# eBay/Sequence-Semantic-Embedding

Measured on AMD Instinct MI355X. Metric: encoded seqs/sec (+ query x target cosine-scores/sec, top-1 vs ref), higher is better.
Workload: dtype f32; 1 GPU; configs[1]: classification stand-in, dual-encoder LSTM H=S=256 E=50 T=32 V=32000; encode 16384 source seqs/GPU/step + cosine top-10 vs 571-target index; batch_per_gpu=16384, seq_len=32, targets=571, parallelism=dp1, weights=random-init (reference initialisers, seed 0)

## Files before the change

### sequence-semantic-embedding_amd/csrc/lstm_fwd.hip

```cpp
#include <cstdlib>
#include <type_traits>

#include "sse_kernels.h"

#define LSTM_THREADS 512
#define LSTM_BM 64

#ifdef SSE_FWD_CLOCK
#include <cstdio>
__device__ long long g_fwd_clk[16 * 8];
#define FW_CLK_DECL long long ck_[8] = {0, 0, 0, 0, 0, 0, 0, 0}, ck_t = clock64();
#define FW_CLK(i)                   \
  {                                 \
    const long long n_ = clock64(); \
    ck_[i] += n_ - ck_t;            \
    ck_t = n_;                      \
  }
#else
#define FW_CLK_DECL
#define FW_CLK(i)
#endif

bool lstm_fwd_x_double(int KGx, int KGh, int RT) { return (size_t)(2 * RT * (KGx + KGh) + 1) * 1024 <= 160 * 1024; }
size_t lstm_fwd_lds_bytes(int KGx, int KGh, int RT) {
  const int xb = lstm_fwd_x_double(KGx, KGh, RT) ? 2 : 1;
  return (size_t)(xb * RT * KGx + 2 * RT * KGh) * 256 * sizeof(float) + 64 * 4 * sizeof(float);
}
static size_t lstm_fwd_xt_lds_bytes(int KGh, int RT) { return (size_t)(2 * RT * KGh) * 256 * sizeof(float) + 64 * 4 * sizeof(float); }


typedef unsigned int u32x4 __attribute__((ext_vector_type(4)));

__device__ __forceinline__ f32x4 wload(__amdgpu_buffer_rsrc_t r, int voff, int soff) {
  return __builtin_bit_cast(f32x4, __builtin_amdgcn_raw_buffer_load_b128(r, voff, soff, 0));
}

struct NoTail {
  __device__ void operator()() const {}
};
template <int MT, bool LIN, bool SWAP, int R = (MT == 1 ? 4 : 3), bool PRIO = true, typename Tail = NoTail>
__device__ __forceinline__ void gemm_pass(__amdgpu_buffer_rsrc_t wr, int voff, int soff, const float *const (&xa)[MT],
                                          const float *const (&ha)[MT], int KGx, int kend, f32x16 (&acc)[MT][2], int kbeg = 0,
                                          const Tail &tail = Tail{}) {
  auto a_frag = [&](int m, int kg) -> f32x4 {
    if constexpr (LIN) return *reinterpret_cast<const f32x4 *>(xa[m] + kg * 256);
    return *reinterpret_cast<const f32x4 *>(kg < KGx ? xa[m] + kg * 256 : ha[m] + (kg - KGx) * 256);
  };
  f32x4 p0[R], p1[R], af[R][MT];
  const int klast = kend - 1;
#pragma unroll
  for (int s = 0; s < R; ++s) {
    const int kg = kbeg + s < kend ? kbeg + s : klast;
    p0[s] = wload(wr, voff, soff + kg * 4096);
    p1[s] = wload(wr, voff + 1024, soff + kg * 4096);
#pragma unroll
    for (int m = 0; m < MT; ++m) af[s][m] = a_frag(m, kg);
    __builtin_amdgcn_sched_barrier(0);
  }
  auto mfmas = [&](int s) {
#pragma unroll
    for (int e = 0; e < 4; ++e)
#pragma unroll
      for (int m = 0; m < MT; ++m) {
        acc[m][0] = SWAP ? __builtin_amdgcn_mfma_f32_32x32x2f32(p0[s][e], af[s][m][e], acc[m][0], 0, 0, 0)
                         : __builtin_amdgcn_mfma_f32_32x32x2f32(af[s][m][e], p0[s][e], acc[m][0], 0, 0, 0);
        acc[m][1] = SWAP ? __builtin_amdgcn_mfma_f32_32x32x2f32(p1[s][e], af[s][m][e], acc[m][1], 0, 0, 0)
                         : __builtin_amdgcn_mfma_f32_32x32x2f32(af[s][m][e], p1[s][e], acc[m][1], 0, 0, 0);
      }
  };
  if constexpr (PRIO) __builtin_amdgcn_s_setprio(1);
  int kg = kbeg;
  for (; kg + R <= kend; kg += R) {
#pragma unroll
    for (int s = 0; s < R; ++s) {
      __builtin_amdgcn_sched_barrier(0);
      mfmas(s);
      __builtin_amdgcn_sched_barrier(0);
      const int kn = (kg + s + R < kend) ? kg + s + R : klast;
      p0[s] = wload(wr, voff, soff + kn * 4096);
      p1[s] = wload(wr, voff + 1024, soff + kn * 4096);
#pragma unroll
      for (int m = 0; m < MT; ++m) af[s][m] = a_frag(m, kn);
    }
  }
  if constexpr (!std::is_same_v<Tail, NoTail>) {
    __builtin_amdgcn_sched_barrier(0);
    tail();
    __builtin_amdgcn_sched_barrier(0);
  }
#pragma unroll
  for (int s = 0; s < R - 1; ++s)
    if (kg + s < kend) mfmas(s);
  if constexpr (PRIO) __builtin_amdgcn_s_setprio(0);
}

template <int RT, int MT, int UBW, bool TRAIN, bool LIN, bool SPL = false, bool TSW = false, bool XT = false>
__global__ __launch_bounds__(LSTM_THREADS) void lstm_fwd_kernel(LstmFwdArgs a) {
  static_assert(!TSW || TRAIN, "TSW is the training forward in the inference orientation");
  static_assert(!XT || (!TRAIN && LIN && !SPL), "the x table is an inference path of the linear LDS layout");
  constexpr int NTHR = LSTM_THREADS;
  extern __shared__ __attribute__((aligned(16))) float smem[];
  constexpr int ROWS = RT * 32;
  constexpr int TPR = NTHR / ROWS;
  constexpr int NWR = 8 / RT;
  constexpr bool SWAP = !TRAIN || TSW;
  const int tid = threadIdx.x, lane = tid & 63, w = tid >> 6;
  const bool split3 = !TRAIN && RT == 2 && MT == 1 && a.H > 64 && a.H <= 96;
  int ub0 = (RT == 2 && MT == 1) ? (w >> 1) : w;
  int mt0 = (RT == 2 && MT == 1) ? (w & 1) : 0;
  bool do_a = true, do_b = true;
  if (split3 && w >= 4) {
    ub0 = 2;
    mt0 = (w - 4) >> 1;
    do_a = ((w & 1) == 0);
    do_b = !do_a;
  }
  if constexpr (SPL) {
    static_assert(RT == 1 && MT == 1 && UBW == 1, "pass-split mapping is defined for one 32-row tile");
    ub0 = w & 3;
    do_a = w < 4;
    do_b = !do_a;
  }
  const int fidx = SPL ? ub0 : mt0;
  const int KGx = a.KGx, KGh = a.KGh, KG = KGx + KGh, T = a.T;
  const int KGhe = (a.KGhe > 0 && a.KGhe < KGh) ? a.KGhe : KGh;
  const int KGxs = XT ? 0 : KGx, KGs = KGxs + KGh;
  constexpr bool XD = LIN;
  auto xptr = [&](int buf, int mt) -> float * {
    return LIN ? smem + (size_t)((buf * RT + mt) * KGs) * 256 : smem + (size_t)(mt * KGx) * 256;
  };
  auto hptr = [&](int buf, int mt) -> float * {
    return LIN ? smem + (size_t)((buf * RT + mt) * KGs + KGxs) * 256
               : smem + (size_t)(RT * KGx + (buf * RT + mt) * KGh) * 256;
  };
  float *red = smem + (size_t)(LIN ? 2 * RT * KGs : RT * KGx + 2 * RT * KGh) * 256;
  const int b0 = blockIdx.x * ROWS;
  int *pass_flag = reinterpret_cast<int *>(red + 16);
  if (tid < 8) pass_flag[tid] = 0;

  const int xr = tid % ROWS, xq = tid / ROWS;
  const bool row_ok = (b0 + xr) < a.B;
  const int32_t *id_row = a.ids + (size_t)(row_ok ? (a.row_map ? a.row_map[b0 + xr] : b0 + xr) : 0) * T;
  auto fetch_id = [&](int t) -> int {
    int id = row_ok ? id_row[t] : 0;
    if (id < 0 || id >= a.V) {
      atomicOr(a.err, 1);
      id = 0;
    }
    return id;
  };
  int xt_row[MT];
#pragma unroll
  for (int m = 0; m < MT; ++m) {
    const int r = b0 + (mt0 + m) * 32 + (lane & 31);
    xt_row[m] = XT && r < a.B ? (a.row_map ? a.row_map[r] : r) : -1;
  }
  auto xt_id = [&](int m, int t) -> int { return xt_row[m] >= 0 ? a.ids[(size_t)xt_row[m] * T + t] : 0; };
  auto xt_check = [&](int id) -> int {
    if (id < 0 || id >= a.V) {
      atomicOr(a.err, 1);
      id = 0;
    }
    return id;
  };
  auto x_store = [&](int buf, int kg, f32x4 lo, f32x4 hi) {
    float *dst = xptr(buf, xr >> 5) + (size_t)kg * 256;
    *reinterpret_cast<f32x4 *>(dst + (xr & 31) * 4) = lo;
    *reinterpret_cast<f32x4 *>(dst + (32 + (xr & 31)) * 4) = hi;
  };

  const int NT32 = a.NT32 > 0 ? a.NT32 : gridDim.x * RT;
  auto tape_x = [&](int ts, int kg, f32x4 lo, f32x4 hi) {
    if constexpr (TSW) {
      if (kg >= 8) return;
      sse_quad_transpose(lo, lane);
      sse_quad_transpose(hi, lane);
      const int KT = 2 + KGh / 4, b = xr & 31;
      const size_t rg = ((size_t)ts * NT32 + blockIdx.x * RT + (xr >> 5)) * 4 + (b >> 3);
      const int k0 = kg * 8 + (xr & 3);
      float *dst = a.tape_a + (rg * KT + (k0 >> 5)) * 256 + ((((b >> 2) & 1) * 32 + (k0 & 31)) << 2);
      __builtin_nontemporal_store(lo, reinterpret_cast<f32x4 *>(dst));
      __builtin_nontemporal_store(hi, reinterpret_cast<f32x4 *>(dst + 16));
    }
  };

  int t0 = 0;
  if (!TRAIN && a.pad_h != nullptr) {
    int lead = T;
    if (row_ok) {
      for (int t = xq; t < T; t += TPR)
        if (id_row[t] != 0) {
          lead = t;
          break;
        }
    }
#pragma unroll
    for (int o = 32; o > 0; o >>= 1) lead = min(lead, __shfl_xor(lead, o));
    if (lane == 0) red[w] = __int_as_float(lead);
    __syncthreads();
    lead = T;
    for (int i = 0; i < NTHR / 64; ++i) lead = min(lead, __float_as_int(red[i]));
    t0 = min(lead, T - 1);
    __syncthreads();
  }

  int xid[MT];
#pragma unroll
  for (int m = 0; m < MT; ++m) xid[m] = XT ? xt_check(xt_id(m, t0)) : 0;
  if constexpr (!XT) {
    const int id = fetch_id(t0);
    const float *src = a.emb + (size_t)id * a.Ep;
    for (int kg = xq; kg < KGx; kg += TPR) {
      f32x4 lo = *reinterpret_cast<const f32x4 *>(src + kg * 8);
      f32x4 hi = *reinterpret_cast<const f32x4 *>(src + kg * 8 + 4);
      x_store(t0 & 1, kg, lo, hi);
    }
    if constexpr (TSW) {
      for (int kg = xq; kg < 8; kg += TPR) {
        f32x4 lo = {0, 0, 0, 0}, hi = {0, 0, 0, 0};
        if (kg < KGx) {
          lo = *reinterpret_cast<const f32x4 *>(src + kg * 8);
          hi = *reinterpret_cast<const f32x4 *>(src + kg * 8 + 4);
        }
        tape_x(t0, kg, lo, hi);
      }
    }
  }
  {
    const int Hp = KGh * 8;
    for (int i = tid; i < RT * KGh * 256; i += NTHR) {
      const int mt = i / (KGh * 256), e = i % (KGh * 256);
      const int un = (e >> 8) * 8 + ((e >> 7) & 1) * 4 + (e & 3);
      hptr(t0 & 1, mt)[e] = (t0 > 0) ? a.pad_h[(size_t)t0 * Hp + un] : 0.0f;
    }
  }

  f32x16 c[UBW][MT];
#pragma unroll
  for (int u = 0; u < UBW; ++u) {
#pragma unroll
    for (int r = 0; r < 16; ++r) {
      const int un = (ub0 + 8 * u) * 32 + (SWAP ? mfma_row(r, lane) : (lane & 31));
      const float c0 = (t0 > 0) ? a.pad_c[(size_t)t0 * (KGh * 8) + un] : 0.0f;
#pragma unroll
      for (int m = 0; m < MT; ++m) c[u][m][r] = c0;
    }
  }

  if constexpr (TSW) {
    if (do_b) {
      const int KT = 2 + KGh / 4, b = lane & 31;
#pragma unroll
      for (int u = 0; u < UBW; ++u)
#pragma unroll
        for (int m = 0; m < MT; ++m) {
          const size_t rg = ((size_t)t0 * NT32 + blockIdx.x * RT + mt0 + m) * 4 + (b >> 3);
#pragma unroll
          for (int q4 = 0; q4 < 4; ++q4) {
            float *dst = a.tape_a + (rg * KT + 2 + ub0 + 8 * u) * 256 + ((((b >> 2) & 1) * 32 + q4 * 8 + (lane >> 5) * 4 + (b & 3)) << 2);
            __builtin_nontemporal_store(f32x4{0, 0, 0, 0}, reinterpret_cast<f32x4 *>(dst));
          }
        }
    }
  }
  __syncthreads();

  const __amdgpu_buffer_rsrc_t wr = __builtin_amdgcn_make_buffer_rsrc(
      const_cast<float *>(a.Wp), 0, (KGh / 4) * KG * 4096, 0x00020000);
  const int wvoff = lane * 16;
  const __amdgpu_buffer_rsrc_t xtr = __builtin_amdgcn_make_buffer_rsrc(
      const_cast<float *>(a.xtab), 0, XT ? a.V * a.xtab_ub * 512 : 0, 0x00020000);
  auto xt_load = [&](f32x16(&acc)[MT][2], const int (&id)[MT], int ub, int q) {
    const int soff = __builtin_amdgcn_readfirstlane(ub * 512 + q * 128);
#pragma unroll
    for (int m = 0; m < MT; ++m) {
      const int voff = id[m] * (a.xtab_ub * 512) + (lane >> 5) * 64;
#pragma unroll
      for (int i = 0; i < 4; ++i) {
        const f32x4 v0 = wload(xtr, voff + 16 * i, soff), v1 = wload(xtr, voff + 128 + 16 * i, soff);
#pragma unroll
        for (int e = 0; e < 4; ++e) {
          acc[m][0][4 * i + e] = v0[e];
          acc[m][1][4 * i + e] = v1[e];
        }
      }
    }
  };

  auto acc_init = [&](f32x16(&acc)[MT][2], const int (&id)[MT], int ub, int q) {
    if constexpr (XT) {
      xt_load(acc, id, ub, q);
    } else {
#pragma unroll
      for (int m = 0; m < MT; ++m)
#pragma unroll
        for (int r = 0; r < 16; ++r) {
          acc[m][0][r] = 0.0f;
          acc[m][1][r] = 0.0f;
        }
    }
  };

  constexpr bool PF = XT && RT == 2 && MT == 2 && UBW == 1;
  const bool live0 = !(a.H > 0 && ub0 * 32 >= a.H);
  f32x16 ga[MT][2], gb[MT][2];
  if (PF && live0) xt_load(ga, xid, ub0, 0);

  FW_CLK_DECL
  for (int t = t0; t < T; ++t) {
    FW_CLK(0)
    const bool have_next = (t + 1) < T;
    int nid = 0;
    f32x4 nlo = {0, 0, 0, 0}, nhi = {0, 0, 0, 0};
    int xnid[MT];
#pragma unroll
    for (int m = 0; m < MT; ++m) xnid[m] = XT && have_next ? xt_id(m, t + 1) : 0;
    if (!XT && have_next) {
      nid = fetch_id(t + 1);
      if (xq < KGx) {
        const float *src = a.emb + (size_t)nid * a.Ep + xq * 8;
        nlo = *reinterpret_cast<const f32x4 *>(src);
        nhi = *reinterpret_cast<const f32x4 *>(src + 4);
      }
    }

    const int cur = t & 1, nxt = (t + 1) & 1;
    const float *xa[MT], *ha[MT];
#pragma unroll
    for (int m = 0; m < MT; ++m) {
      xa[m] = xptr(cur, mt0 + m) + lane * 4;
      ha[m] = hptr(cur, mt0 + m) + lane * 4;
    }

    if constexpr (TRAIN && !TSW) {
      const int KT = 2 + KGh / 4;
      const int nk = 64 + KGh * 8;
      auto a_elem = [&](int mt, int kp, int b) -> float {
        if (kp >= 64) {
          const int un = kp - 64;
          return hptr(cur, mt)[(size_t)(un >> 3) * 256 + ((((un >> 2) & 1) * 32 + b) << 2) + (un & 3)];
        }
        if (kp < KGx * 8) return xptr(cur, mt)[(size_t)(kp >> 3) * 256 + ((((kp >> 2) & 1) * 32 + b) << 2) + (kp & 3)];
        return 0.0f;
      };
      if (a.tape_a_split) {
        unsigned short *ta = reinterpret_cast<unsigned short *>(a.tape_a);
        for (int i = tid; i < nk * (ROWS / 8); i += NTHR) {
          const int kp = i % nk, o = i / nk;
          const int mt = o >> 2, oc = o & 3;
          float v8[8];
#pragma unroll
          for (int e = 0; e < 8; ++e) v8[e] = a_elem(mt, kp, oc * 8 + e);
          sse_u32x4 hi, lo;
          sse_split8(v8, hi, lo);
          const size_t g16 = ((size_t)t * NT32 + blockIdx.x * RT + mt) * 2 + (oc >> 1);
          unsigned short *dst = ta + ((g16 * KT + (kp >> 5)) * 2) * 512 + ((oc & 1) * 32 + (kp & 31)) * 8;
          *reinterpret_cast<sse_u32x4 *>(dst) = hi;
          *reinterpret_cast<sse_u32x4 *>(dst + 512) = lo;
        }
      } else {
        for (int i = tid; i < nk * (ROWS / 4); i += NTHR) {
          const int kp = i % nk, b4 = i / nk;
          const int mt = b4 >> 3, bl = (b4 & 7) * 4;
          const f32x4 v = {a_elem(mt, kp, bl), a_elem(mt, kp, bl + 1), a_elem(mt, kp, bl + 2), a_elem(mt, kp, bl + 3)};
          const size_t rg = ((size_t)t * NT32 + blockIdx.x * RT + mt) * 4 + (bl >> 3);
          float *dst = a.tape_a + (rg * KT + (kp >> 5)) * 256 + ((((bl >> 2) & 1) * 32 + (kp & 31)) << 2);
          *reinterpret_cast<f32x4 *>(dst) = v;
        }
      }
    }
    const int kend = (t == 0) ? KGx : KGx + KGhe;

#pragma unroll
    for (int u = 0; u < UBW; ++u) {
      const int ub = ub0 + 8 * u;
      if (!TRAIN && a.H > 0 && ub * 32 >= a.H) {
        if (u == 0 && XD && !XT && have_next) {
          if (xq < KGx) x_store(nxt, xq, nlo, nhi);
          for (int kg = xq + TPR; kg < KGx; kg += TPR) {
            const float *src = a.emb + (size_t)nid * a.Ep + kg * 8;
            x_store(nxt, kg, *reinterpret_cast<const f32x4 *>(src), *reinterpret_cast<const f32x4 *>(src + 4));
          }
        }
        continue;
      }
      const int unit = ub * 32 + (lane & 31);
      const int hoff = SWAP ? (ub * 4) * 256 + lane * 4
                            : (unit >> 3) * 256 + ((((unit >> 2) & 1) * 32) << 2) + (unit & 3);
      const int wsoff = __builtin_amdgcn_readfirstlane(ub) * KG * 4096;
      float *tp[MT];
      if constexpr (TRAIN) {
#pragma unroll
        for (int m = 0; m < MT; ++m)
          tp[m] = a.tape_g + (((size_t)t * NT32 + blockIdx.x * RT + mt0 + m) * (KGh / 4) + ub) * 5 * 1024 + lane * 4;
      }

      float *hdst[MT];
      auto pass = [&](int soff, f32x16(&acc)[MT][2], const auto &tail) {
        if constexpr (XT) {
          if (t > 0) gemm_pass<MT, true, SWAP>(wr, wvoff, soff + KGx * 4096, ha, ha, 0, KGhe, acc, 0, tail);
          else tail();
        } else {
          gemm_pass<MT, LIN, SWAP>(wr, wvoff, soff, xa, ha, KGx, kend, acc);
        }
      };
      auto tail_a = [&] {
        if constexpr (PF) xt_load(gb, xid, ub, 2);
      };
      auto tail_b = [&] {
        if constexpr (PF) {
          if (u + 1 < UBW && (a.H <= 0 || (ub + 8) * 32 < a.H)) {
            xt_load(ga, xid, ub + 8, 0);
          } else if (have_next) {
#pragma unroll
            for (int m = 0; m < MT; ++m) xid[m] = xt_check(xnid[m]);
            xt_load(ga, xid, ub0, 0);
          } else {
#pragma unroll
            for (int m = 0; m < MT; ++m)
#pragma unroll
              for (int r = 0; r < 16; ++r) ga[m][0][r] = ga[m][1][r] = 0.0f;
          }
        }
      };
#pragma unroll
      for (int m = 0; m < MT; ++m) hdst[m] = hptr(nxt, mt0 + m) + hoff;
      if (!PF && (!XT || do_a)) acc_init(ga, xid, ub, 0);
      FW_CLK(1)
      if (do_a) pass(wsoff, ga, tail_a);
      FW_CLK(2)
#pragma unroll
      for (int m = 0; m < MT; ++m) {
        if (!do_a) break;
        if constexpr (SWAP) {
#pragma unroll
          for (int q4 = 0; q4 < 4; ++q4) {
            f32x4 pij, si4, tj4;
#pragma unroll
            for (int e = 0; e < 4; ++e) {
              si4[e] = sse_sigmoid(ga[m][0][q4 * 4 + e]);
              tj4[e] = sse_tanh(ga[m][1][q4 * 4 + e]);
              pij[e] = si4[e] * tj4[e];
            }
            *reinterpret_cast<f32x4 *>(hdst[m] + q4 * 256) = pij;
            if constexpr (TSW) {
              __builtin_nontemporal_store(si4, reinterpret_cast<f32x4 *>(tp[m] + q4 * 256));
              __builtin_nontemporal_store(tj4, reinterpret_cast<f32x4 *>(tp[m] + 1024 + q4 * 256));
            }
          }
        } else {
#pragma unroll
          for (int q4 = 0; q4 < 4; ++q4) {
            f32x4 si4, tj4;
#pragma unroll
            for (int e = 0; e < 4; ++e) {
              const int r = q4 * 4 + e;
              si4[e] = sse_sigmoid(ga[m][0][r]);
              tj4[e] = sse_tanh(ga[m][1][r]);
              hdst[m][mfma_row(r, lane) << 2] = si4[e] * tj4[e];
            }
            if constexpr (TRAIN) {
              __builtin_nontemporal_store(si4, reinterpret_cast<f32x4 *>(tp[m] + q4 * 256));
              __builtin_nontemporal_store(tj4, reinterpret_cast<f32x4 *>(tp[m] + 1024 + q4 * 256));
            }
          }
        }
      }
      if (do_a && !do_b) {
        __builtin_amdgcn_s_waitcnt(0xc07f);
        if (lane == 0) __hip_atomic_store(pass_flag + fidx, t + 1, __ATOMIC_RELAXED, __HIP_MEMORY_SCOPE_WORKGROUP);
      }
      if (u == 0 && XD && !XT && have_next) {
        if (xq < KGx) x_store(nxt, xq, nlo, nhi);
        for (int kg = xq + TPR; kg < KGx; kg += TPR) {
          const float *src = a.emb + (size_t)nid * a.Ep + kg * 8;
          x_store(nxt, kg, *reinterpret_cast<const f32x4 *>(src), *reinterpret_cast<const f32x4 *>(src + 4));
        }
        tape_x(t + 1, xq, nlo, nhi);
      }
      if (!PF && (!XT || do_b)) acc_init(gb, xid, ub, 2);
      FW_CLK(3)
      if (do_b) pass(wsoff + 2048, gb, tail_b);
      FW_CLK(4)
      if (do_b && !do_a) {
        while (__hip_atomic_load(pass_flag + fidx, __ATOMIC_RELAXED, __HIP_MEMORY_SCOPE_WORKGROUP) < t + 1) __builtin_amdgcn_s_sleep(2);
        asm volatile("" ::: "memory");
      }
      FW_CLK(5)
#pragma unroll
      for (int m = 0; m < MT; ++m) {
        if (!do_b) break;
        if constexpr (SWAP) {
#pragma unroll
          for (int q4 = 0; q4 < 4; ++q4) {
            const f32x4 pij = *reinterpret_cast<const f32x4 *>(hdst[m] + q4 * 256);
            f32x4 hv4;
#pragma unroll
            for (int e = 0; e < 4; ++e) {
              const int r = q4 * 4 + e;
              const float sf = sse_sigmoid(gb[m][0][r]);
              const float so = sse_sigmoid(gb[m][1][r]);
              const float cn = c[u][m][r] * sf + pij[e];
              c[u][m][r] = cn;
              hv4[e] = sse_tanh(cn) * so;
              if (a.rec_h != nullptr && blockIdx.x == 0 && mt0 + m == 0 && (lane & 31) == 0) {
                a.rec_h[(size_t)(t + 1) * (KGh * 8) + ub * 32 + mfma_row(r, lane)] = hv4[e];
                a.rec_c[(size_t)(t + 1) * (KGh * 8) + ub * 32 + mfma_row(r, lane)] = cn;
              }
            }
            *reinterpret_cast<f32x4 *>(hdst[m] + q4 * 256) = hv4;
            if constexpr (TSW) {
              f32x4 sf4, so4, cn4;
#pragma unroll
              for (int e = 0; e < 4; ++e) {
                const int r = q4 * 4 + e;
                sf4[e] = sse_sigmoid(gb[m][0][r]);
                so4[e] = sse_sigmoid(gb[m][1][r]);
                cn4[e] = c[u][m][r];
              }
              __builtin_nontemporal_store(sf4, reinterpret_cast<f32x4 *>(tp[m] + 2048 + q4 * 256));
              __builtin_nontemporal_store(so4, reinterpret_cast<f32x4 *>(tp[m] + 3072 + q4 * 256));
              __builtin_nontemporal_store(cn4, reinterpret_cast<f32x4 *>(tp[m] + 4096 + q4 * 256));
              if (have_next) {
                f32x4 ht = hv4;
                sse_quad_transpose(ht, lane);
                const int KT = 2 + KGh / 4, b = lane & 31;
                const size_t rg = ((size_t)(t + 1) * NT32 + blockIdx.x * RT + mt0 + m) * 4 + (b >> 3);
                float *dst = a.tape_a + (rg * KT + 2 + ub) * 256 + ((((b >> 2) & 1) * 32 + q4 * 8 + (lane >> 5) * 4 + (b & 3)) << 2);
                __builtin_nontemporal_store(ht, reinterpret_cast<f32x4 *>(dst));
              }
            }
          }
        } else {
#pragma unroll
          for (int q4 = 0; q4 < 4; ++q4) {
            f32x4 sf4, so4, cn4;
#pragma unroll
            for (int e = 0; e < 4; ++e) {
              const int r = q4 * 4 + e;
              const float sf = sse_sigmoid(gb[m][0][r]);
              const float so = sse_sigmoid(gb[m][1][r]);
              const float cn = c[u][m][r] * sf + hdst[m][mfma_row(r, lane) << 2];
              c[u][m][r] = cn;
              const float hv = sse_tanh(cn) * so;
              hdst[m][mfma_row(r, lane) << 2] = hv;
              sf4[e] = sf;
              so4[e] = so;
              cn4[e] = cn;
            }
            if constexpr (TRAIN) {
              __builtin_nontemporal_store(sf4, reinterpret_cast<f32x4 *>(tp[m] + 2048 + q4 * 256));
              __builtin_nontemporal_store(so4, reinterpret_cast<f32x4 *>(tp[m] + 3072 + q4 * 256));
              __builtin_nontemporal_store(cn4, reinterpret_cast<f32x4 *>(tp[m] + 4096 + q4 * 256));
            }
          }
        }
      }
    }

    FW_CLK(6)
    if (XD) {
      __syncthreads();
      FW_CLK(7)
#pragma unroll
      for (int m = 0; m < MT; ++m)
        if (XT && !(PF && live0) && have_next) xid[m] = xt_check(xnid[m]);
    } else {
      __syncthreads();
      if (have_next) {
        if (xq < KGx) x_store(0, xq, nlo, nhi);
        for (int kg = xq + TPR; kg < KGx; kg += TPR) {
          const float *src = a.emb + (size_t)nid * a.Ep + kg * 8;
          x_store(0, kg, *reinterpret_cast<const f32x4 *>(src), *reinterpret_cast<const f32x4 *>(src + 4));
        }
        tape_x(t + 1, xq, nlo, nhi);
      }
      __syncthreads();
    }
  }

#ifdef SSE_FWD_CLOCK
  if (blockIdx.x == 0 && lane == 0)
    for (int i = 0; i < 8; ++i) g_fwd_clk[w * 8 + i] = ck_[i];
#endif
  if constexpr (TRAIN) {
    const int Hp = KGh * 8;
    for (int i = tid; i < ROWS * Hp; i += NTHR) {
      const int un = i % Hp, b = i / Hp;
      a.h_last[(size_t)(b0 + b) * Hp + un] =
          hptr(T & 1, b >> 5)[(size_t)(un >> 3) * 256 + ((((un >> 2) & 1) * 32 + (b & 31)) << 2) + (un & 3)];
    }
  }

  const int wn = w % NWR, wm = w / NWR;
  constexpr bool pwave = true;
  constexpr int PT = 16 / NWR;
  const float *hp = hptr(T & 1, wm) + lane * 4;
  f32x16 pacc[PT];
  float *ssq = hptr((T + 1) & 1, 0);
#pragma unroll
  for (int i = 0; i < PT; ++i) {
    const int nt = wn + NWR * i;
#pragma unroll
    for (int r = 0; r < 16; ++r) pacc[i][r] = 0.0f;
    if (nt < a.NTS && pwave) {
      const float *mp = a.Mp + (size_t)nt * KGh * 256 + lane * 4;
      f32x4 ax = *reinterpret_cast<const f32x4 *>(hp), bx = *reinterpret_cast<const f32x4 *>(mp), ay, by;
      int kg = 0;
      for (; kg + 1 < KGhe; kg += 2) {
        ay = *reinterpret_cast<const f32x4 *>(hp + (kg + 1) * 256);
        by = *reinterpret_cast<const f32x4 *>(mp + (kg + 1) * 256);
        __builtin_amdgcn_sched_barrier(0);
#pragma unroll
        for (int e = 0; e < 4; ++e) pacc[i] = __builtin_amdgcn_mfma_f32_32x32x2f32(ax[e], bx[e], pacc[i], 0, 0, 0);
        __builtin_amdgcn_sched_barrier(0);
        const int k2 = (kg + 2 < KGhe) ? kg + 2 : kg;
        ax = *reinterpret_cast<const f32x4 *>(hp + k2 * 256);
        bx = *reinterpret_cast<const f32x4 *>(mp + k2 * 256);
        __builtin_amdgcn_sched_barrier(0);
#pragma unroll
        for (int e = 0; e < 4; ++e) pacc[i] = __builtin_amdgcn_mfma_f32_32x32x2f32(ay[e], by[e], pacc[i], 0, 0, 0);
        __builtin_amdgcn_sched_barrier(0);
      }
      if (kg < KGhe) {
#pragma unroll
        for (int e = 0; e < 4; ++e) pacc[i] = __builtin_amdgcn_mfma_f32_32x32x2f32(ax[e], bx[e], pacc[i], 0, 0, 0);
      }
      if (a.normalize) {
#pragma unroll
        for (int r = 0; r < 16; ++r) {
          float v = pacc[i][r] * pacc[i][r];
          v += __shfl_xor(v, 1);
          v += __shfl_xor(v, 2);
          v += __shfl_xor(v, 4);
          v += __shfl_xor(v, 8);
          v += __shfl_xor(v, 16);
          if ((lane & 31) == 0) ssq[(wm * 32 + mfma_row(r, lane)) * 16 + nt] = v;
        }
      }
    }
  }
  float scale[16];
  if (a.normalize) {
    __syncthreads();
#pragma unroll
    for (int r = 0; r < 16; ++r) {
      const float *pr = ssq + (wm * 32 + mfma_row(r, lane)) * 16;
      float tot = 0.0f;
      for (int j = 0; j < a.NTS; ++j) tot += pr[j];
      scale[r] = 1.0f / sqrtf(fmaxf(tot, 1e-12f));
    }
  } else {
#pragma unroll
    for (int r = 0; r < 16; ++r) scale[r] = 1.0f;
  }
#pragma unroll
  for (int i = 0; i < PT; ++i) {
    const int nt = wn + NWR * i;
    const int col = nt * 32 + (lane & 31);
    if (nt < a.NTS && col < a.S && pwave) {
#pragma unroll
      for (int r = 0; r < 16; ++r) {
        const int row = b0 + wm * 32 + mfma_row(r, lane);
        if (row < a.B) a.out[(size_t)(a.row_map ? a.row_map[row] : row) * a.S + col] = pacc[i][r] * scale[r];
      }
    }
  }
}

template <int RT, int MT, int UBW, bool TRAIN, bool LIN, bool SPL, bool TSW = false, bool XT = false>
static hipError_t launch_one(const LstmFwdArgs &a, size_t lds, hipStream_t stream) {
  hipError_t e = hipFuncSetAttribute(reinterpret_cast<const void *>(lstm_fwd_kernel<RT, MT, UBW, TRAIN, LIN, SPL, TSW, XT>),
                                     hipFuncAttributeMaxDynamicSharedMemorySize, (int)lds);
  if (e != hipSuccess) return e;
  const dim3 grid(a.NT32 > 0 ? a.NT32 / RT : (a.B + RT * 32 - 1) / (RT * 32)), block(LSTM_THREADS);
  hipLaunchKernelGGL((lstm_fwd_kernel<RT, MT, UBW, TRAIN, LIN, SPL, TSW, XT>), grid, block, lds, stream, a);
#ifdef SSE_FWD_CLOCK
  {
    static int n = 0;
    if (a.B >= 1024 && n++ % 16 == 4) {
      long long v[128];
      (void)hipStreamSynchronize(stream);
      (void)hipMemcpyFromSymbol(v, HIP_SYMBOL(g_fwd_clk), sizeof v);
      for (int w = 0; w < 8; ++w)
        fprintf(stderr, "[fwd clock <%d,%d,%d> B=%d H=%d] wave %d cycles/step: prefetch %lld | setup %lld | passA gemm %lld | epiA+x %lld | passB gemm %lld | flag wait %lld | epiB %lld | barrier %lld\n",
                RT, MT, UBW, a.B, a.H, w, v[w * 8 + 0] / a.T, v[w * 8 + 1] / a.T, v[w * 8 + 2] / a.T, v[w * 8 + 3] / a.T, v[w * 8 + 4] / a.T, v[w * 8 + 5] / a.T,
                v[w * 8 + 6] / a.T, v[w * 8 + 7] / a.T);
    }
  }
#endif
  return hipGetLastError();
}

template <int RT, int MT, int UBW, bool SPL = false>
static hipError_t launch_cfg(const LstmFwdArgs &a_in, hipStream_t stream) {
  LstmFwdArgs a = a_in;
  a.xdouble = lstm_fwd_x_double(a.KGx, a.KGh, RT) ? 1 : 0;
  const size_t lds = lstm_fwd_lds_bytes(a.KGx, a.KGh, RT);
  const bool train = a.tape_g != nullptr;
  if constexpr (!SPL && !(RT == 2 && MT == 1)) {
    if (!train && a.xtab != nullptr) {
      if (a.xtab_ub != (a.H > 0 ? (a.H + 31) / 32 : a.KGh / 4)) return hipErrorInvalidValue;
      if ((int64_t)a.V * a.xtab_ub * 512 > INT32_MAX) return hipErrorInvalidValue;
      return launch_one<RT, MT, UBW, false, true, false, false, true>(a, lstm_fwd_xt_lds_bytes(a.KGh, RT), stream);
    }
  }
  if (train && a.tape_swap) {
    if (a.tape_a_split) return hipErrorInvalidValue;
    return a.xdouble ? launch_one<RT, MT, UBW, true, true, SPL, true>(a, lds, stream)
                     : launch_one<RT, MT, UBW, true, false, SPL, true>(a, lds, stream);
  }
  if (a.xdouble)
    return train ? launch_one<RT, MT, UBW, true, true, SPL>(a, lds, stream) : launch_one<RT, MT, UBW, false, true, SPL>(a, lds, stream);
  return train ? launch_one<RT, MT, UBW, true, false, SPL>(a, lds, stream) : launch_one<RT, MT, UBW, false, false, SPL>(a, lds, stream);
}

int lstm_fwd_rows_per_wg(int Hp, int B, int tiles_elsewhere, int cus) {
  if (cus <= 0) cus = 256;
  if (Hp == 512) return 32;
  if ((Hp == 256 || Hp == 128) && (B + 31) / 32 + tiles_elsewhere <= cus) return 32;
  if (tiles_elsewhere == 0 && (Hp == 256 || Hp == 128)) {
    const int n64 = (B + 63) / 64, n32 = (B + 31) / 32;
    const double full = Hp == 256 ? 1.006 : 1.06;
    const int rem = n32 % (2 * cus);
    const double t64 = (double)((n64 + cus - 1) / cus), t32 = (n32 / (2 * cus)) * full + (rem == 0 ? 0.0 : rem <= cus ? 0.55 : full);
    if (t32 < 0.93 * t64) return 32;
  }
  return 64;
}

int lstm_fwd_variant(const LstmFwdArgs &a, int Hp) {
  int rows = lstm_fwd_rows_per_wg(Hp, a.B, a.tiles_elsewhere, a.cu_count);
  if (Hp <= 256 && (a.force_rows == 32 || a.force_rows == 64)) rows = a.force_rows;
  if (const char *ev = getenv("SSE_FWD_ROWS")) {
    const int r = atoi(ev);
    if (Hp <= 256 && (r == 32 || r == 64)) rows = r;
  }
  if (Hp == 128 && rows == 64 && a.gate_split && a.tape_g == nullptr && a.rec_h == nullptr && a.NTS <= 16 &&
      lstm_fwd_gs_ok(a.KGx, a.KGh, a.H > 0 ? a.H : Hp)) {
    const char *ev = getenv("SSE_FWD_GS");
    if (!(ev && atoi(ev) == 0)) return rows | LSTM_FWD_GATE_SPLIT;
  }
  return rows | (Hp != 128 && a.tape_g == nullptr && a.xtab != nullptr ? LSTM_FWD_X_TABLE : 0);
}

hipError_t launch_lstm_fwd(const LstmFwdArgs &a, int Hp, hipStream_t stream) {
  const int variant = lstm_fwd_variant(a, Hp), rows = variant & (32 | 64);
  if (rows == 64 && a.NT32 > 0 && (a.NT32 & 1)) return hipErrorInvalidValue;
  if (Hp == 128 && a.xtab != nullptr) return hipErrorInvalidValue;
  if (variant & LSTM_FWD_GATE_SPLIT) {
    LstmFwdArgs g = a;
    if (g.H <= 0) g.H = Hp;
    return launch_lstm_fwd_gs(g, stream);
  }
  if (Hp == 128) return rows == 32 ? launch_cfg<1, 1, 1, true>(a, stream) : launch_cfg<2, 1, 1>(a, stream);
  if (Hp == 256) return rows == 32 ? launch_cfg<1, 1, 1>(a, stream) : launch_cfg<2, 2, 1>(a, stream);
  if (Hp == 512) return launch_cfg<1, 1, 2>(a, stream);
  return hipErrorInvalidValue;
}
```

Measured before the change: 7.578 million seqs/s.

## Overlap x-table prefetch with pad scan and pipeline projection epilogue

Moves the x-table id lookup and first gate prefetch ahead of the leading-pad reduction barrier, so the global load latency overlaps the scan. It also simplifies the initial h fill, zeroing with vector stores when t0 is 0. The projection epilogue is restructured: each wave handles all row tiles for its target column tiles, runs a 4-deep buffer-load pipeline for the projection weights, batches the norm shuffles, and hoists row_map lookups. Debug timeline instrumentation is added under the clock macro. The change adds register pressure and hardcodes the column-tile mapping to 8 waves with two tiles each.

```diff
diff --git a/sequence-semantic-embedding_amd/csrc/lstm_fwd.hip b/sequence-semantic-embedding_amd/csrc/lstm_fwd.hip
--- a/sequence-semantic-embedding_amd/csrc/lstm_fwd.hip
+++ b/sequence-semantic-embedding_amd/csrc/lstm_fwd.hip
@@ -16,9 +16,14 @@
     ck_[i] += n_ - ck_t;            \
     ck_t = n_;                      \
   }
+#define FW_TL_MAX 4096
+__device__ long long g_fwd_tl[FW_TL_MAX * 5];
+#define FW_TL(i) \
+  if (threadIdx.x == 0 && blockIdx.x < FW_TL_MAX) g_fwd_tl[blockIdx.x * 5 + (i)] = wall_clock64();
 #else
 #define FW_CLK_DECL
 #define FW_CLK(i)
+#define FW_TL(i)
 #endif
 
 bool lstm_fwd_x_double(int KGx, int KGh, int RT) { return (size_t)(2 * RT * (KGx + KGh) + 1) * 1024 <= 160 * 1024; }
@@ -102,9 +107,9 @@
   extern __shared__ __attribute__((aligned(16))) float smem[];
   constexpr int ROWS = RT * 32;
   constexpr int TPR = NTHR / ROWS;
-  constexpr int NWR = 8 / RT;
   constexpr bool SWAP = !TRAIN || TSW;
   const int tid = threadIdx.x, lane = tid & 63, w = tid >> 6;
+  FW_TL(0)
   const bool split3 = !TRAIN && RT == 2 && MT == 1 && a.H > 64 && a.H <= 96;
   int ub0 = (RT == 2 && MT == 1) ? (w >> 1) : w;
   int mt0 = (RT == 2 && MT == 1) ? (w & 1) : 0;
@@ -184,9 +189,36 @@
     }
   };
 
+  const __amdgpu_buffer_rsrc_t xtr = __builtin_amdgcn_make_buffer_rsrc(
+      const_cast<float *>(a.xtab), 0, XT ? a.V * a.xtab_ub * 512 : 0, 0x00020000);
+  auto xt_load = [&](f32x16(&acc)[MT][2], const int (&id)[MT], int ub, int q) {
+    const int soff = __builtin_amdgcn_readfirstlane(ub * 512 + q * 128);
+#pragma unroll
+    for (int m = 0; m < MT; ++m) {
+      const int voff = id[m] * (a.xtab_ub * 512) + (lane >> 5) * 64;
+#pragma unroll
+      for (int i = 0; i < 4; ++i) {
+        const f32x4 v0 = wload(xtr, voff + 16 * i, soff), v1 = wload(xtr, voff + 128 + 16 * i, soff);
+#pragma unroll
+        for (int e = 0; e < 4; ++e) {
+          acc[m][0][4 * i + e] = v0[e];
+          acc[m][1][4 * i + e] = v1[e];
+        }
+      }
+    }
+  };
+  constexpr bool PF = XT && RT == 2 && MT == 2 && UBW == 1;
+  const bool live0 = !(a.H > 0 && ub0 * 32 >= a.H);
+  f32x16 ga[MT][2], gb[MT][2];
+
+  int xid[MT];
+#pragma unroll
+  for (int m = 0; m < MT; ++m) xid[m] = XT ? xt_id(m, 0) : 0;
+
   int t0 = 0;
-  if (!TRAIN && a.pad_h != nullptr) {
-    int lead = T;
+  const bool scan = !TRAIN && a.pad_h != nullptr;
+  int lead = T;
+  if (scan) {
     if (row_ok) {
       for (int t = xq; t < T; t += TPR)
         if (id_row[t] != 0) {
@@ -196,6 +228,13 @@
     }
 #pragma unroll
     for (int o = 32; o > 0; o >>= 1) lead = min(lead, __shfl_xor(lead, o));
+  }
+  if constexpr (XT) {
+#pragma unroll
+    for (int m = 0; m < MT; ++m) xid[m] = xt_check(xid[m]);
+    if (PF && live0) xt_load(ga, xid, ub0, 0);
+  }
+  if (scan) {
     if (lane == 0) red[w] = __int_as_float(lead);
     __syncthreads();
     lead = T;
@@ -204,9 +243,11 @@
     __syncthreads();
   }
 
-  int xid[MT];
-#pragma unroll
-  for (int m = 0; m < MT; ++m) xid[m] = XT ? xt_check(xt_id(m, t0)) : 0;
+  if (XT && t0 > 0) {
+#pragma unroll
+    for (int m = 0; m < MT; ++m) xid[m] = xt_check(xt_id(m, t0));
+    if (PF && live0) xt_load(ga, xid, ub0, 0);
+  }
   if constexpr (!XT) {
     const int id = fetch_id(t0);
     const float *src = a.emb + (size_t)id * a.Ep;
@@ -226,12 +267,18 @@
       }
     }
   }
-  {
-    const int Hp = KGh * 8;
-    for (int i = tid; i < RT * KGh * 256; i += NTHR) {
-      const int mt = i / (KGh * 256), e = i % (KGh * 256);
-      const int un = (e >> 8) * 8 + ((e >> 7) & 1) * 4 + (e & 3);
-      hptr(t0 & 1, mt)[e] = (t0 > 0) ? a.pad_h[(size_t)t0 * Hp + un] : 0.0f;
+  if (t0 == 0) {
+#pragma unroll
+    for (int mt = 0; mt < RT; ++mt) {
+      f32x4 *dst = reinterpret_cast<f32x4 *>(hptr(0, mt));
+      for (int i = tid; i < KGh * 64; i += NTHR) dst[i] = f32x4{0.0f, 0.0f, 0.0f, 0.0f};
+    }
+  } else {
+    const float *ph = a.pad_h + (size_t)t0 * (KGh * 8);
+    for (int e = tid; e < KGh * 256; e += NTHR) {
+      const float v = ph[(e >> 8) * 8 + ((e >> 7) & 1) * 4 + (e & 3)];
+#pragma unroll
+      for (int mt = 0; mt < RT; ++mt) hptr(t0 & 1, mt)[e] = v;
     }
   }
 
@@ -268,24 +315,6 @@
   const __amdgpu_buffer_rsrc_t wr = __builtin_amdgcn_make_buffer_rsrc(
       const_cast<float *>(a.Wp), 0, (KGh / 4) * KG * 4096, 0x00020000);
   const int wvoff = lane * 16;
-  const __amdgpu_buffer_rsrc_t xtr = __builtin_amdgcn_make_buffer_rsrc(
-      const_cast<float *>(a.xtab), 0, XT ? a.V * a.xtab_ub * 512 : 0, 0x00020000);
-  auto xt_load = [&](f32x16(&acc)[MT][2], const int (&id)[MT], int ub, int q) {
-    const int soff = __builtin_amdgcn_readfirstlane(ub * 512 + q * 128);
-#pragma unroll
-    for (int m = 0; m < MT; ++m) {
-      const int voff = id[m] * (a.xtab_ub * 512) + (lane >> 5) * 64;
-#pragma unroll
-      for (int i = 0; i < 4; ++i) {
-        const f32x4 v0 = wload(xtr, voff + 16 * i, soff), v1 = wload(xtr, voff + 128 + 16 * i, soff);
-#pragma unroll
-        for (int e = 0; e < 4; ++e) {
-          acc[m][0][4 * i + e] = v0[e];
-          acc[m][1][4 * i + e] = v1[e];
-        }
-      }
-    }
-  };
 
   auto acc_init = [&](f32x16(&acc)[MT][2], const int (&id)[MT], int ub, int q) {
     if constexpr (XT) {
@@ -301,12 +330,9 @@
     }
   };
 
-  constexpr bool PF = XT && RT == 2 && MT == 2 && UBW == 1;
-  const bool live0 = !(a.H > 0 && ub0 * 32 >= a.H);
-  f32x16 ga[MT][2], gb[MT][2];
-  if (PF && live0) xt_load(ga, xid, ub0, 0);
 
   FW_CLK_DECL
+  FW_TL(1)
   for (int t = t0; t < T; ++t) {
     FW_CLK(0)
     const bool have_next = (t + 1) < T;
@@ -579,6 +605,7 @@
     }
   }
 
+  FW_TL(2)
 #ifdef SSE_FWD_CLOCK
   if (blockIdx.x == 0 && lane == 0)
     for (int i = 0; i < 8; ++i) g_fwd_clk[w * 8 + i] = ck_[i];
@@ -592,80 +619,134 @@
     }
   }
 
-  const int wn = w % NWR, wm = w / NWR;
-  constexpr bool pwave = true;
-  constexpr int PT = 16 / NWR;
-  const float *hp = hptr(T & 1, wm) + lane * 4;
-  f32x16 pacc[PT];
+  constexpr int PT = 2;
+  constexpr int PR = 4;
+  const float *hp[RT];
+#pragma unroll
+  for (int m = 0; m < RT; ++m) hp[m] = hptr(T & 1, m) + lane * 4;
+  const __amdgpu_buffer_rsrc_t mr = __builtin_amdgcn_make_buffer_rsrc(const_cast<float *>(a.Mp), 0, a.NTS * KGh * 1024, 0x00020000);
+  f32x16 pacc[PT][RT];
   float *ssq = hptr((T + 1) & 1, 0);
 #pragma unroll
   for (int i = 0; i < PT; ++i) {
-    const int nt = wn + NWR * i;
-#pragma unroll
-    for (int r = 0; r < 16; ++r) pacc[i][r] = 0.0f;
-    if (nt < a.NTS && pwave) {
-      const float *mp = a.Mp + (size_t)nt * KGh * 256 + lane * 4;
-      f32x4 ax = *reinterpret_cast<const f32x4 *>(hp), bx = *reinterpret_cast<const f32x4 *>(mp), ay, by;
+    const int nt = __builtin_amdgcn_readfirstlane(w) + 8 * i;
+#pragma unroll
+    for (int m = 0; m < RT; ++m)
+#pragma unroll
+      for (int r = 0; r < 16; ++r) pacc[i][m][r] = 0.0f;
+    if (nt < a.NTS) {
+      const int msoff = nt * KGh * 1024, klast = KGhe - 1;
+      f32x4 bm[PR], ah[PR][RT];
+      auto fill = [&](int s, int kg) {
+        bm[s] = wload(mr, wvoff, msoff + kg * 1024);
+#pragma unroll
+        for (int m = 0; m < RT; ++m) ah[s][m] = *reinterpret_cast<const f32x4 *>(hp[m] + kg * 256);
+      };
+      auto mfmas = [&](int s) {
+#pragma unroll
+        for (int e = 0; e < 4; ++e)
+#pragma unroll
+          for (int m = 0; m < RT; ++m) pacc[i][m] = __builtin_amdgcn_mfma_f32_32x32x2f32(ah[s][m][e], bm[s][e], pacc[i][m], 0, 0, 0);
+      };
+#pragma unroll
+      for (int s = 0; s < PR; ++s) {
+        fill(s, s < KGhe ? s : klast);
+        __builtin_amdgcn_sched_barrier(0);
+      }
       int kg = 0;
-      for (; kg + 1 < KGhe; kg += 2) {
-        ay = *reinterpret_cast<const f32x4 *>(hp + (kg + 1) * 256);
-        by = *reinterpret_cast<const f32x4 *>(mp + (kg + 1) * 256);
-        __builtin_amdgcn_sched_barrier(0);
-#pragma unroll
-        for (int e = 0; e < 4; ++e) pacc[i] = __builtin_amdgcn_mfma_f32_32x32x2f32(ax[e], bx[e], pacc[i], 0, 0, 0);
-        __builtin_amdgcn_sched_barrier(0);
-        const int k2 = (kg + 2 < KGhe) ? kg + 2 : kg;
-        ax = *reinterpret_cast<const f32x4 *>(hp + k2 * 256);
-        bx = *reinterpret_cast<const f32x4 *>(mp + k2 * 256);
-        __builtin_amdgcn_sched_barrier(0);
-#pragma unroll
-        for (int e = 0; e < 4; ++e) pacc[i] = __builtin_amdgcn_mfma_f32_32x32x2f32(ay[e], by[e], pacc[i], 0, 0, 0);
-        __builtin_amdgcn_sched_barrier(0);
-      }
-      if (kg < KGhe) {
-#pragma unroll
-        for (int e = 0; e < 4; ++e) pacc[i] = __builtin_amdgcn_mfma_f32_32x32x2f32(ax[e], bx[e], pacc[i], 0, 0, 0);
-      }
+      for (; kg + PR <= KGhe; kg += PR) {
+#pragma unroll
+        for (int s = 0; s < PR; ++s) {
+          __builtin_amdgcn_sched_barrier(0);
+          mfmas(s);
+          __builtin_amdgcn_sched_barrier(0);
+          fill(s, kg + s + PR < KGhe ? kg + s + PR : klast);
+        }
+      }
+#pragma unroll
+      for (int s = 0; s < PR - 1; ++s)
+        if (kg + s < KGhe) mfmas(s);
       if (a.normalize) {
-#pragma unroll
-        for (int r = 0; r < 16; ++r) {
-          float v = pacc[i][r] * pacc[i][r];
-          v += __shfl_xor(v, 1);
-          v += __shfl_xor(v, 2);
-          v += __shfl_xor(v, 4);
-          v += __shfl_xor(v, 8);
-          v += __shfl_xor(v, 16);
-          if ((lane & 31) == 0) ssq[(wm * 32 + mfma_row(r, lane)) * 16 + nt] = v;
-        }
-      }
-    }
-  }
-  float scale[16];
+        float v[RT][16];
+#pragma unroll
+        for (int m = 0; m < RT; ++m)
+#pragma unroll
+          for (int r = 0; r < 16; ++r) {
+            const float x = pacc[i][m][r];
+            v[m][r] = __builtin_fmaf(x, x, __shfl_xor(x * x, 1));
+          }
+#pragma unroll
+        for (int o = 2; o <= 16; o <<= 1)
+#pragma unroll
+          for (int m = 0; m < RT; ++m)
+#pragma unroll
+            for (int r = 0; r < 16; ++r) v[m][r] += __shfl_xor(v[m][r], o);
+        if ((lane & 31) == 0) {
+#pragma unroll
+          for (int m = 0; m < RT; ++m)
+#pragma unroll
+            for (int r = 0; r < 16; ++r) ssq[(m * 32 + mfma_row(r, lane)) * 16 + nt] = v[m][r];
+        }
+      }
+    }
+  }
+  float scale[RT][16];
   if (a.normalize) {
     __syncthreads();
-#pragma unroll
-    for (int r = 0; r < 16; ++r) {
-      const float *pr = ssq + (wm * 32 + mfma_row(r, lane)) * 16;
-      float tot = 0.0f;
-      for (int j = 0; j < a.NTS; ++j) tot += pr[j];
-      scale[r] = 1.0f / sqrtf(fmaxf(tot, 1e-12f));
-    }
+    const float *pr = ssq + (lane % ROWS) * 16;
+    float tot = 0.0f;
+    for (int j = 0; j < a.NTS; ++j) tot += pr[j];
+    const float sc = 1.0f / sqrtf(fmaxf(tot, 1e-12f));
+#pragma unroll
+    for (int m = 0; m < RT; ++m)
+#pragma unroll
+      for (int r = 0; r < 16; ++r) scale[m][r] = __shfl(sc, m * 32 + mfma_row(r, lane));
   } else {
 #pragma unroll
-    for (int r = 0; r < 16; ++r) scale[r] = 1.0f;
+    for (int m = 0; m < RT; ++m)
+#pragma unroll
+      for (int r = 0; r < 16; ++r) scale[m][r] = 1.0f;
+  }
+  int orow[RT][16];
+#pragma unroll
+  for (int m = 0; m < RT; ++m)
+#pragma unroll
+    for (int r = 0; r < 16; ++r) orow[m][r] = b0 + m * 32 + mfma_row(r, lane);
+  if (a.row_map != nullptr) {
+#pragma unroll
+    for (int m = 0; m < RT; ++m)
+#pragma unroll
+      for (int r = 0; r < 16; ++r) {
+        const int mapped = a.row_map[min(orow[m][r], a.B - 1)];
+        orow[m][r] = orow[m][r] < a.B ? mapped : -1;
+      }
+  } else {
+#pragma unroll
+    for (int m = 0; m < RT; ++m)
+#pragma unroll
+      for (int r = 0; r < 16; ++r) orow[m][r] = orow[m][r] < a.B ? orow[m][r] : -1;
   }
 #pragma unroll
   for (int i = 0; i < PT; ++i) {
-    const int nt = wn + NWR * i;
+    const int nt = w + 8 * i;
     const int col = nt * 32 + (lane & 31);
-    if (nt < a.NTS && col < a.S && pwave) {
-#pragma unroll
-      for (int r = 0; r < 16; ++r) {
-        const int row = b0 + wm * 32 + mfma_row(r, lane);
-        if (row < a.B) a.out[(size_t)(a.row_map ? a.row_map[row] : row) * a.S + col] = pacc[i][r] * scale[r];
-      }
-    }
-  }
+    if (nt < a.NTS && col < a.S) {
+#pragma unroll
+      for (int m = 0; m < RT; ++m)
+#pragma unroll
+        for (int r = 0; r < 16; ++r)
+          if (orow[m][r] >= 0) a.out[(size_t)orow[m][r] * a.S + col] = pacc[i][m][r] * scale[m][r];
+    }
+  }
+#ifdef SSE_FWD_CLOCK
+  asm volatile("s_waitcnt vmcnt(0)" ::: "memory");
+  FW_TL(3)
+  if (tid == 0 && blockIdx.x < FW_TL_MAX) {
+    int xcc;
+    asm volatile("s_getreg_b32 %0, hwreg(HW_REG_XCC_ID)" : "=s"(xcc));
+    g_fwd_tl[blockIdx.x * 5 + 4] = xcc & 15;
+  }
+#endif
 }
 
 template <int RT, int MT, int UBW, bool TRAIN, bool LIN, bool SPL, bool TSW = false, bool XT = false>
@@ -686,6 +767,14 @@
         fprintf(stderr, "[fwd clock <%d,%d,%d> B=%d H=%d] wave %d cycles/step: prefetch %lld | setup %lld | passA gemm %lld | epiA+x %lld | passB gemm %lld | flag wait %lld | epiB %lld | barrier %lld\n",
                 RT, MT, UBW, a.B, a.H, w, v[w * 8 + 0] / a.T, v[w * 8 + 1] / a.T, v[w * 8 + 2] / a.T, v[w * 8 + 3] / a.T, v[w * 8 + 4] / a.T, v[w * 8 + 5] / a.T,
                 v[w * 8 + 6] / a.T, v[w * 8 + 7] / a.T);
+      if (getenv("SSE_FWD_TIMELINE")) {
+        static long long tl[FW_TL_MAX * 5];
+        const int nwg = (int)grid.x < FW_TL_MAX ? (int)grid.x : FW_TL_MAX;
+        (void)hipMemcpyFromSymbol(tl, HIP_SYMBOL(g_fwd_tl), (size_t)nwg * 5 * sizeof(long long));
+        for (int g = 0; g < nwg; ++g)
+          fprintf(stderr, "[fwd timeline <%d,%d,%d> B=%d] wg %d xcc %lld entry %lld first %lld exit %lld last %lld\n", RT, MT, UBW, a.B, g,
+                  tl[g * 5 + 4], tl[g * 5], tl[g * 5 + 1], tl[g * 5 + 2], tl[g * 5 + 3]);
+      }
     }
   }
 #endif
```

After: 7.577 million seqs/s, median of 2. Within noise of the previous version (-0.0%).
